# heat1q/libldpc

Measured on AMD Instinct MI355X. Metric: decoded frames/s (n=1024 code, 50 BP iters, AWGN), higher is better.
Workload: dtype f64

## Files before the change

include/ldpc_amd.h:

```cpp
#ifndef LDPC_AMD_H
#define LDPC_AMD_H

#include <stdbool.h>
#include <stdint.h>

#ifdef __cplusplus
extern "C" {
#endif

#if defined(__GNUC__)
#pragma GCC visibility push(default)
#endif

typedef struct
{
    bool earlyTerm;
    uint32_t iterations;
    const char *type;
} decoder_param;

typedef struct
{
    uint64_t seed;
    double xRange[3];
// ... 259 lines not shown
int ldpc_hip_mt64(ldpc_hip_ctx *ctx, uint64_t seed, uint64_t first, uint64_t n, uint64_t *out, void *hip_stream);

int ldpc_hip_selftest_division(ldpc_hip_ctx *ctx, uint64_t n, uint64_t seed, uint64_t *mismatches);

int ldpc_hip_selftest_math(ldpc_hip_ctx *ctx, int fn, uint64_t n, const double *a, const double *b, double *out);

uint64_t ldpc_hip_selftest_chunk_table(uint64_t first_chunk, uint64_t chunks_per_request, uint64_t n_requests, uint64_t gap);
uint64_t ldpc_hip_selftest_shard_table(int world, int rank, uint32_t piece_chunks, uint64_t steps, uint64_t *launches);
uint64_t ldpc_hip_jump_tasks(const ldpc_hip_ctx *ctx);

int ldpc_hip_simulate(ldpc_hip_ctx *ctx, decoder_param dec, channel_param ch, simulation_param sim,
                      sim_results_t *results, uint64_t *totals, bool *stopFlag, int cli_output);

typedef struct ldpc_hip_comm ldpc_hip_comm;

int ldpc_hip_comm_unique_id(uint8_t id[128]);
ldpc_hip_comm *ldpc_hip_comm_create(int rank, int world, int device, const uint8_t id[128]);
ldpc_hip_comm *ldpc_hip_comm_create_shm(int rank, int world, const char *name);
ldpc_hip_comm *ldpc_hip_comm_create_echo(int rank, int world);
void ldpc_hip_comm_destroy(ldpc_hip_comm *comm);
int ldpc_hip_comm_allgather(ldpc_hip_comm *comm, const void *send, void *recv, uint64_t bytes);
void ldpc_hip_fused_plan_info(const ldpc_hip_ctx *ctx, int64_t info[8]);
int ldpc_hip_fused_program(const ldpc_hip_ctx *ctx);
int ldpc_hip_decode_stages(const ldpc_hip_ctx *ctx, decoder_param dec, int32_t stages[3]);
int ldpc_hip_decoder_choice(const ldpc_hip_ctx *ctx, decoder_param dec);
int ldpc_hip_selftest_sim_fold(const uint32_t *iters, const uint32_t *bit_errors, uint64_t n, const uint64_t *ends,
                               uint64_t n_ranges, int world, uint64_t min_fec, uint64_t max_frames, uint64_t out[8]);
int ldpc_hip_selftest_layer_plan(ldpc_hip_ctx *ctx, int32_t *step_of_row);
int ldpc_hip_selftest_place(ldpc_hip_comm *comm, uint64_t nct, uint64_t pairs_before, uint64_t frame_pos, uint64_t cap,
                            uint64_t piece_pairs, uint64_t pairs_with_margin, uint64_t status, uint64_t out[5]);
void ldpc_hip_comm_stats(ldpc_hip_comm *comm, double out[4], int reset);
const char *ldpc_hip_comm_describe(ldpc_hip_comm *comm);

uint64_t ldpc_hip_shard_capacity(const ldpc_hip_ctx *ctx, uint64_t target_frames, int world);
int ldpc_hip_stream_decode_sharded(ldpc_hip_ctx *ctx, ldpc_hip_comm *comm, decoder_param dec, uint64_t target_frames,
                                   const ldpc_hip_out *out, uint64_t step[4], void *hip_stream);
int ldpc_hip_simulate_sharded(ldpc_hip_ctx *ctx, ldpc_hip_comm *comm, decoder_param dec, channel_param ch,
                              simulation_param sim, sim_results_t *results, uint64_t *totals, bool *stopFlag,
                              int cli_output);

#if defined(__GNUC__)
#pragma GCC visibility pop
#endif

#ifdef __cplusplus
}
// ... 3 lines not shown
```

libldpc_amd/binding.py:

```python
import ctypes as ct
import os

import numpy as np

PKG = os.path.dirname(os.path.abspath(__file__))
LIB_PATH = os.environ.get("LDPC_AMD_LIB") or os.path.join(PKG, "libldpc.so")

AWGN, BSC, BEC = 1, 2, 3
CHANNELS = {"AWGN": AWGN, "BSC": BSC, "BEC": BEC}


class decoder_param(ct.Structure):
    _fields_ = [("earlyTerm", ct.c_bool), ("iterations", ct.c_uint32), ("type", ct.c_char_p)]


class channel_param(ct.Structure):
    _fields_ = [("seed", ct.c_uint64), ("xRange", ct.c_double * 3), ("type", ct.c_char_p)]


class simulation_param(ct.Structure):
    _fields_ = [("threads", ct.c_uint32), ("maxFrames", ct.c_uint64), ("fec", ct.c_uint64),
                ("resultFile", ct.c_char_p)]


# ... 148 lines not shown
    L.ldpc_hip_synchronize.argtypes = [vp, vp]
    L.ldpc_hip_batch_counters.restype = i32
    L.ldpc_hip_batch_counters.argtypes = [vp, vp, vp, u64, ct.c_uint32, i32, vp, vp]
    L.ldpc_hip_selftest_division.restype = i32
    L.ldpc_hip_selftest_division.argtypes = [vp, u64, u64, vp]
    L.ldpc_hip_mt64.restype = i32
    L.ldpc_hip_mt64.argtypes = [vp, u64, u64, u64, vp, vp]
    L.ldpc_hip_set_profiling.argtypes = [vp, i32]
    L.ldpc_hip_last_ms.restype = ct.c_float
    L.ldpc_hip_last_ms.argtypes = [vp, i32]
    L.ldpc_hip_comm_unique_id.restype = i32
    L.ldpc_hip_comm_unique_id.argtypes = [vp]
    L.ldpc_hip_comm_create.restype = vp
    L.ldpc_hip_comm_create.argtypes = [i32, i32, i32, vp]
    L.ldpc_hip_comm_create_shm.restype = vp
    L.ldpc_hip_comm_create_shm.argtypes = [i32, i32, ct.c_char_p]
    L.ldpc_hip_comm_create_echo.restype = vp
    L.ldpc_hip_comm_create_echo.argtypes = [i32, i32]
    L.ldpc_hip_comm_destroy.argtypes = [vp]
    L.ldpc_hip_comm_allgather.restype = i32
    L.ldpc_hip_comm_allgather.argtypes = [vp, vp, vp, u64]
    L.ldpc_hip_fused_plan_info.restype = None
    L.ldpc_hip_fused_plan_info.argtypes = [vp, vp]
    L.ldpc_hip_fused_program.restype = i32
    L.ldpc_hip_fused_program.argtypes = [vp]
    L.ldpc_hip_decode_stages.restype = i32
    L.ldpc_hip_decode_stages.argtypes = [vp, decoder_param, vp]
    L.ldpc_hip_decoder_choice.restype = i32
    L.ldpc_hip_decoder_choice.argtypes = [vp, decoder_param]
    L.ldpc_hip_selftest_sim_fold.restype = i32
    L.ldpc_hip_selftest_sim_fold.argtypes = [vp, vp, u64, vp, u64, i32, u64, u64, vp]
    L.ldpc_hip_selftest_layer_plan.restype = i32
    L.ldpc_hip_selftest_layer_plan.argtypes = [vp, vp]
    L.ldpc_hip_selftest_place.restype = i32
    L.ldpc_hip_selftest_place.argtypes = [vp, u64, u64, u64, u64, u64, u64, u64, vp]
    L.ldpc_hip_comm_stats.restype = None
    L.ldpc_hip_comm_stats.argtypes = [vp, vp, i32]
    L.ldpc_hip_comm_describe.restype = ct.c_char_p
    L.ldpc_hip_comm_describe.argtypes = [vp]
    L.ldpc_hip_shard_capacity.restype = u64
    L.ldpc_hip_shard_capacity.argtypes = [vp, u64, i32]
    L.ldpc_hip_stream_decode_sharded.restype = i32
    L.ldpc_hip_stream_decode_sharded.argtypes = [vp, vp, decoder_param, u64, ct.POINTER(ldpc_hip_out), vp, vp]
    L.ldpc_hip_simulate_sharded.restype = i32
    L.ldpc_hip_simulate_sharded.argtypes = [vp, vp, decoder_param, channel_param, simulation_param, ct.POINTER(sim_results_t),
                                            vp, ct.POINTER(ct.c_bool), i32]
# ... 114 lines not shown
            self.ctx = None

    __del__ = close

    def _check(self, rc, what):
        if rc != 0:
            raise RuntimeError(f"{what}: " + self.lib.ldpc_hip_last_error().decode())

    def _outs(self, n, want, out):
        bufs = dict(out or {})
        for name in want:
            if name not in bufs:
                dt, per_bit = self.OUT_SPEC[name]
                bufs[name] = np.zeros((n, self.nc) if per_bit else (n,), dt)
        s = ldpc_hip_out(*[_ptr(bufs.get(k)) for k in ("iters", "bit_errors", "hard", "llr_out", "llr_in", "codeword")])
        return s, bufs

    def set_bec_compat(self, on):
        self.lib.ldpc_hip_set_bec_compat(self.ctx, int(on))

    def fused_plan(self):
        info = (ct.c_int64 * 8)()
        self.lib.ldpc_hip_fused_plan_info(self.ctx, info)
        return dict(zip(("ok", "n_slots", "vnb", "cnl", "small", "calls_stride", "has_shortened", "table_entries"), [int(v) for v in info]))

    def fused_program(self):
        return int(self.lib.ldpc_hip_fused_program(self.ctx))

    STAGES = ("whole", "ratio-first", "ratio-separate", "list-chain", "llr-redo", "handover-first", "handover-resume")

    def decode_stages(self, early_term=True, iterations=50, decoding="BP"):
        stages = (ct.c_int32 * 3)()
        n = self.lib.ldpc_hip_decode_stages(self.ctx, _dec(early_term, iterations, decoding), stages)
        return [self.STAGES[stages[i]] for i in range(n)]

    DECODERS = ("resident", "fast32", "layered32", "layered16", "layered-min-sum", "quantized-min-sum", "ternary",
                "layered-fixed-min-sum")

    def decoder_choice(self, early_term=True, iterations=50, decoding="BP"):
        return self.DECODERS[self.lib.ldpc_hip_decoder_choice(self.ctx, _dec(early_term, iterations, decoding))]

    def set_fast_mode(self, on):
        self.lib.ldpc_hip_set_fast_mode(self.ctx, int(on))

    NOISE_MODES = {"reference": 0, "counter": 1}

    def set_noise(self, mode):
# ... 524 lines not shown
```

libldpc_amd/csrc/api.cpp:

```cpp
#include "../../include/ldpc_amd.h"

#include <hip/hip_runtime.h>

#include <algorithm>
#include <cstdio>
#include <cstdlib>
#include <cstring>
#include <iostream>
#include <memory>
#include <string>
#include <vector>

#include "engine.hpp"
#include "shard_place.hpp"
#include "sim.hpp"
#include "sim_fold.hpp"

using namespace ldpc_amd;

struct ldpc_hip_comm
{
    std::unique_ptr<Comm> comm;
    std::string description;
};
// ... 872 lines not shown
    return c;
}

void ldpc_hip_comm_destroy(ldpc_hip_comm *comm) { delete comm; }

int ldpc_hip_comm_allgather(ldpc_hip_comm *comm, const void *send, void *recv, uint64_t bytes)
{
    return guarded([&] { comm->comm->all_gather(send, recv, bytes); });
}

void ldpc_hip_fused_plan_info(const ldpc_hip_ctx *ctx, int64_t info[8])
{
    const FusedPlan &f = ctx->eng->fused_plan();
    info[0] = f.ok ? 1 : 0, info[1] = f.n_slots, info[2] = f.vnb, info[3] = f.cnl, info[4] = f.wide_exclusive ? 1 : 0;
    info[5] = f.calls_stride, info[6] = f.has_shortened ? 1 : 0, info[7] = static_cast<int64_t>(f.vn_slot.size());
}

int ldpc_hip_fused_program(const ldpc_hip_ctx *ctx)
{
    const FusedPlan &f = ctx->eng->fused_plan();
    return f.ok ? f.program : -1;
}

int ldpc_hip_decode_stages(const ldpc_hip_ctx *ctx, decoder_param dec, int32_t stages[3])
{
    const StageSeq seq = ctx->eng->stages(to_params(dec));
    for (int i = 0; i < seq.n; ++i)
        stages[i] = static_cast<int32_t>(seq.s[i]);
    return seq.n;
}

int ldpc_hip_decoder_choice(const ldpc_hip_ctx *ctx, decoder_param dec) { return static_cast<int>(ctx->eng->decoder(to_params(dec))); }

int ldpc_hip_selftest_layer_plan(ldpc_hip_ctx *ctx, int32_t *step_of_row)
{
    if (!step_of_row)
        return ctx->eng->layer_plan_builds();
    int n = -1;
    if (guarded([&] {
            const LayerPlan &L = ctx->eng->layer_plan();
            if (!L.ok)
                throw std::runtime_error("the layered schedule does not take this code");
            for (size_t i = 0; i < L.step_of_row.size(); ++i)
                step_of_row[i] = L.step_of_row[i];
            n = static_cast<int>(L.steps.size());
        }) != 0)
// ... 101 lines not shown
```

libldpc_amd/csrc/fused_program.hpp:

```cpp
#pragma once

#include <cstdint>

#include "plan.hpp"

namespace ldpc_amd
{

constexpr int kFusedProgCalls = 2;

struct FusedProgCall
{
    int degree, leaf, nm;
    uint32_t cnt0, cnt1;
    uint32_t off0, off1;
    constexpr bool two() const { return cnt1 != 0; }
    constexpr uint32_t flip() const { return ((1u << nm) - 1u) << (degree - leaf - nm); }
    constexpr uint32_t cls() const { return static_cast<uint32_t>(degree) | (static_cast<uint32_t>(leaf) << 3) | (flip() << 4); }
    constexpr FusedCall call() const { return cnt0 ? FusedCall{off0 | (off1 << 16), cnt0 | (cnt1 << 16), cls(), 0} : FusedCall{0, 0, 0, 0}; }
    constexpr bool valid() const { return cnt0 == 0 || (cnt0 <= kWaveSize && (cnt1 == 0 || (cnt0 == kWaveSize && cnt1 == kWaveSize))); }
};

struct FusedProgWave
{
    FusedProgCall leaf;
    FusedProgCall calls[kFusedProgCalls];
    uint32_t vn_kind[4], vn_cnt[4], vn_deg[4];
    constexpr uint32_t vn_prog() const { return vn_kind[0] | (vn_kind[1] << 4) | (vn_kind[2] << 8) | (vn_kind[3] << 12); }
    constexpr uint32_t vn_desc(int s) const { return vn_kind[s] == kFusedVnNone ? 0u : (vn_cnt[s] | (vn_deg[s] << 16)); }
};

struct FusedProgram
{
    int n_slots, vnb, cnl;
    FusedProgWave wave[kDecodeWaves];
};

namespace fused_program_detail
{
constexpr uint32_t kB = kWaveSize * 8u;
constexpr FusedProgCall pair(int d, int leaf, int nm, uint32_t first_slot_byte)
{
    return FusedProgCall{d, leaf, nm, kWaveSize, kWaveSize, first_slot_byte, first_slot_byte + static_cast<uint32_t>(d - leaf) * kB};
}
constexpr FusedProgCall none() { return FusedProgCall{0, 0, 0, 0, 0, 0, 0}; }
constexpr FusedProgWave wide_wave(FusedProgCall leaf, FusedProgCall rest, uint32_t dv)
{
    return FusedProgWave{leaf, {rest, none()}, {kFusedVnWide, kFusedVnNone, kFusedVnNone, kFusedVnNone}, {kWaveSize, 0, 0, 0}, {dv, 0, 0, 0}};
}
constexpr FusedProgWave pairs_wave(FusedProgCall leaf, FusedProgCall rest)
{
    return FusedProgWave{leaf, {rest, none()}, {kFusedVnPair, kFusedVnPair, kFusedVnPair, kFusedVnPair}, {kWaveSize, kWaveSize, kWaveSize, kWaveSize}, {2, 2, 2, 2}};
}
}

constexpr FusedProgram kFusedPrograms[] = {
    {2944, 4, 1,
     {fused_program_detail::wide_wave(fused_program_detail::pair(4, 1, 0, 2048), fused_program_detail::pair(3, 0, 2, 14336), 15),
      fused_program_detail::wide_wave(fused_program_detail::pair(4, 1, 0, 5120), fused_program_detail::pair(3, 0, 2, 17408), 15),
      fused_program_detail::pairs_wave(fused_program_detail::pair(4, 1, 0, 8192), fused_program_detail::pair(3, 0, 2, 20480)),
      fused_program_detail::pairs_wave(fused_program_detail::pair(3, 1, 0, 0), fused_program_detail::pair(3, 0, 2, 11264))}},
};
constexpr int kNumFusedPrograms = static_cast<int>(sizeof(kFusedPrograms) / sizeof(kFusedPrograms[0]));

constexpr bool fused_program_valid(const FusedProgram &p)
{
    if (p.vnb > 4 || p.cnl > 1 || static_cast<uint32_t>(p.n_slots) * 8u > 0x10000u)
        return false;
    for (const FusedProgWave &w : p.wave)
    {
        if (!w.leaf.valid() || (w.leaf.cnt0 != 0 && (w.leaf.leaf != 1 || w.leaf.degree < 3 || w.leaf.degree > 4)))
            return false;
        for (const FusedProgCall &c : w.calls)
            if (!c.valid() || (c.cnt0 != 0 && (c.leaf != 0 || c.degree < 2 || c.degree > 4)))
                return false;
        const bool wide = w.vn_kind[0] == kFusedVnWide;
        for (int s = 0; s < 4; ++s)
        {
            const uint32_t k = w.vn_kind[s];
            if (k == kFusedVnWide ? (s != 0 || w.vn_deg[s] < 3 || w.vn_deg[s] > 15 || w.vn_cnt[s] == 0 || w.vn_cnt[s] > kWaveSize)
                                  : (k == kFusedVnPair ? (w.vn_deg[s] != 2 || w.vn_cnt[s] != kWaveSize || w.vn_kind[s ^ 1] != kFusedVnPair)
                                                       : (k == kFusedVn2 ? (w.vn_deg[s] != 2 || w.vn_cnt[s] == 0 || w.vn_cnt[s] >= kWaveSize) : k != kFusedVnNone)))
                return false;
            if (wide && s > 0 && k != kFusedVnNone)
// ... 18 lines not shown
```

libldpc_amd/csrc/kernels_fused.hip:

```cpp
#include <hip/hip_runtime.h>

#include <algorithm>
#include <utility>

#include "device_cn.hpp"
#include "device_math.hpp"
#include "device_philox.hpp"
#include "fused_program.hpp"
#include "fused_rule.h"
#include "kernels.hpp"
#include "launch_lds.hpp"

#ifndef LDPC_AMD_DECODE_PRIO
#define LDPC_AMD_DECODE_PRIO 3
#endif
#ifndef LDPC_AMD_FUSED_WAVES
#define LDPC_AMD_FUSED_WAVES 6
#endif

namespace ldpc_amd
{

namespace
{

constexpr int kThreads = kDecodeWaves * kWaveSize;

__device__ __forceinline__ double *at(char *msg, uint32_t byte_off) { return reinterpret_cast<double *>(msg + byte_off); }

struct Track
{
    uint32_t hmax, hmin, pmax;
};
__device__ __forceinline__ void track(Track &t, double a)
{
    t.hmax = max(t.hmax, hi_word(a));
    t.hmin = min(t.hmin, hi_word(a));
}
__device__ __forceinline__ void track2(Track &t, double a, double b)
{
    t.hmax = max(max(t.hmax, hi_word(a)), hi_word(b));
    t.hmin = min(min(t.hmin, hi_word(a)), hi_word(b));
}

template <int D, bool LEAF, unsigned FLIP, bool TWO, bool WANT_TOT, bool SHARED = true>
__device__ __forceinline__ uint32_t cnf_call(char *msg, uint32_t off0, uint32_t off1, uint32_t cnt0, int lane, double rho0, double rho1,
                                             uint32_t prev0, uint32_t prev1, uint32_t &lb0, uint32_t &lb1, Track &t, double &tot0,
                                             double &tot1)
{
    constexpr int M = D - (LEAF ? 1 : 0);
    const uint32_t stride = TWO ? kWaveSize * 8u : cnt0 * 8u;
// ... 622 lines not shown
            else
            {
                if (k01 & 0xFu)
                    one(w, k01 & 0xFu);
                if (k01 >> 4)
                    one(w + 1, k01 >> 4);
            }
        }
        vn_bits = bits;
    };
    [[maybe_unused]] auto prog_cn = [&]<int W, int C>() {
        if constexpr (PROG >= 0)
        {
            constexpr FusedProgCall k = C < 0 ? kFusedPrograms[PROG].wave[W].leaf : kFusedPrograms[PROG].wave[W].calls[C];
            if constexpr (k.cnt0 != 0)
            {
                constexpr bool LEAF = C < 0;
                uint32_t lb0 = 0, lb1 = 0, par = 0;
                double tot0 = 1.0, tot1 = 1.0;
                const uint32_t prev0 = LEAF ? leaf_bits << 31 : 0u, prev1 = LEAF ? leaf_bits << 30 : 0u;
                const double rho0 = LEAF ? leaf_rho[0] : 0.0, rho1 = LEAF ? leaf_rho[1] : 0.0;
                if constexpr (k.two())
                    par = cnf_call<k.degree, LEAF, k.flip(), true, false>(msg, k.off0, k.off1, k.cnt0, lane, rho0, rho1, prev0, prev1, lb0, lb1, t, tot0, tot1);
                else if (lane < static_cast<int>(k.cnt0))
                    par = cnf_call<k.degree, LEAF, k.flip(), false, false>(msg, k.off0, 0, k.cnt0, lane, rho0, rho1, prev0, prev1, lb0, lb1, t, tot0, tot1);
                bad |= par;
                if constexpr (LEAF)
                    new_leaf_bits |= lb0 | (lb1 << 1);
            }
        }
    };
    [[maybe_unused]] auto prog_cn_wave = [&]<int W>() { prog_cn.template operator()<W, -1>(), prog_cn.template operator()<W, 0>(), prog_cn.template operator()<W, 1>(); };
    [[maybe_unused]] auto prog_vn2 = [&]<int W, int S>() {
        if constexpr (PROG >= 0)
        {
            constexpr FusedProgWave pw = kFusedPrograms[PROG].wave[W];
            if constexpr (pw.vn_kind[S] == kFusedVnPair && pw.vn_kind[S + 1] == kFusedVnPair)
            {
                uint32_t sga, sgb;
                double ta, tb;
                vn2_pair(msg, idx_at(S), idx_at(S + 1), val_at(S), val_at(S + 1), t, sga, sgb, ta, tb);
                bits |= ((sga >> 31) << S) | ((sgb >> 31) << (S + 1));
            }
            else
            {
#pragma unroll
                for (int s = S; s < S + 2; ++s)
// ... 131 lines not shown
                    }
                };
                for (int c = 0; c < CNL; ++c)
                    if ((leaf_calls_now[4 * c + 1] & 0xFFFFu) != 0)
                        ho_call(leaf_calls_now[4 * c], leaf_calls_now[4 * c + 1], leaf_calls_now[4 * c + 2], c);
                for (int c = 0; c < F.calls_stride; ++c)
                {
                    if ((my_calls[4 * c + 1] & 0xFFFFu) == 0)
                        break;
                    ho_call(my_calls[4 * c], my_calls[4 * c + 1], my_calls[4 * c + 2], 0);
                }
                return;
            }
            cn_pass();
            commit_leaves();
            __syncthreads();
            vn_pass();
            post_vote(I + 1);
            __syncthreads();
            ++I;
        }
    }
    else
    for (;;)
    {
        loop_cn_pass();
        const int ph = I & 1;
        const bool esc = dm_box_escaped(t.hmax, t.hmin) || t.pmax >= DM_FUSED_P_HI;
        const int wave_vote = (__ballot((bad & 0x80000000u) != 0) != 0) | ((__ballot(esc) != 0) << 1);
        if (lane == 0)
            votes[ph][wave] = wave_vote;
        __syncthreads();
        int any = 0;
#pragma unroll
        for (int w = 0; w < kDecodeWaves; ++w)
            any |= votes[ph][w];
        if (any & 2)
        {
            if (tid == 0)
            {
                const uint32_t pos = atomicAdd(a.redo_count, 1u);
                a.redo_list[pos] = static_cast<uint32_t>(frame);
            }
            return;
        }
        if (I > 0 && a.early_term && !(any & 1))
        {
            --I;
            break;
        }
        if (I == a.iterations)
            break;
        commit_leaves();

        loop_vn_pass();
        __syncthreads();
        ++I;
    }

    if (tid == 0 && a.iters)
        a.iters[frame] = I;
    uint8_t *hard = a.hard ? a.hard + frame * nc : nullptr;
    int err = 0;
    if (hard || a.bit_errors)
    {
        int lane_now = lane;
        asm volatile("" : "+v"(lane_now));
        const uint32_t *tab = F.lane_tab + (static_cast<uint32_t>(wave) * kFusedLaneRows) * kWaveSize + lane_now;
        auto account = [&](uint32_t cwd, uint32_t bit) {
            if (cwd == kFusedNone)
                return;
            const uint32_t col = cwd & 0x3FFFFFFFu;
            if (hard)
                hard[col] = static_cast<uint8_t>(bit);
            if (cwd & kFusedCounted)
                err += static_cast<int>(bit) != (cw ? static_cast<int>(cw[col]) : 0);
        };
#pragma unroll
        for (int w = 0; w < VNB; ++w)
            account(tab[(24 + w) * kWaveSize], (vn_bits >> w) & 1u);
// ... 501 lines not shown
```

libldpc_amd/csrc/plan.cpp:

```cpp
#include "plan.hpp"

#include "fused_program.hpp"
#include "fused_rule.h"

#include <algorithm>
#include <cstdio>
#include <cstdlib>
#include <map>
#include <numeric>
#include <stdexcept>

#ifndef LDPC_AMD_FUSED_PROGRAM
#define LDPC_AMD_FUSED_PROGRAM 1
#endif

namespace ldpc_amd
{

namespace
{
void deal(const std::vector<int> &cost, std::vector<uint32_t> &work, int &stride)
{
    std::vector<int> order(cost.size());
    std::iota(order.begin(), order.end(), 0);
// ... 403 lines not shown
        }
    }
    r.uniform_cn = std::all_of(r.cn_deg.begin(), r.cn_deg.end(), [&](uint8_t d) { return d == maxd; });
    r.uniform_vn = nv0 >= 2 && nv1 >= 2;
    for (int rd = 0; rd < 2 && r.uniform_vn; ++rd)
    {
        const int nvr = rd ? nv1 : nv0;
        auto blk = [&](int q) -> const Reg2VnBlock & { return r.vn_blocks[static_cast<size_t>(q / W + (rd ? nv0 : 0)) * W + q % W]; };
        const Reg2VnBlock &b0 = blk(0), &b1 = blk(1);
        uint32_t *af = r.vn_affine[rd];
        af[0] = b0.p0_off, af[1] = b1.p0_off - b0.p0_off, af[2] = b0.prest_off, af[3] = b1.prest_off - b0.prest_off;
        af[4] = b0.tot_off, af[5] = b1.tot_off - b0.tot_off;
        for (int q = 0; q < nvr * W && r.uniform_vn; ++q)
        {
            const Reg2VnBlock &b = blk(q);
            r.uniform_vn = b.count == kWaveSize && b.degree == 3 && b.p0_off == af[0] + af[1] * q && b.prest_off == af[2] + af[3] * q &&
                           b.tot_off == af[4] + af[5] * q;
        }
    }
    r.ok = true;
    return r;
}

FusedPlan build_fused_plan(const LdpcCode &code, const Plan &plan)
{
    FusedPlan f;
    const SparseGF2 &H = code.H;
    if (!plan.lds_ok || plan.has_isolated_vn || H.rows <= 0 ||
        !dm_fused_applies(H.rows, H.cols, H.rptr.data(), H.rcol.data(), H.cptr.data()))
        return f;
    const int W = kDecodeWaves;
    static_assert(DM_FUSED_MAX_LEAF_CALLS == kDecodeWaves * kFusedLeafCalls && DM_FUSED_MAX_VN_BLOCKS == kDecodeWaves * kFusedVnSlots,
                  "a code the rule admits has a plan: the oracle decides by the rule alone");
    auto cdeg = [&](int c) { return H.cptr[c + 1] - H.cptr[c]; };

    struct Row
    {
        int row, order[4];
    };
    std::map<unsigned, std::vector<Row>> by_class;
    for (int i = 0; i < H.rows; ++i)
    {
        Row r{i, {0, 0, 0, 0}};
        unsigned flip;
        int leaf;
        const int d = H.rptr[i + 1] - H.rptr[i];
// ... 13 lines not shown
    for (auto &[cls, rows] : by_class)
    {
        const int d = static_cast<int>(cls & 7u), leaf = static_cast<int>((cls >> 3) & 1u), m = d - leaf;
        for (size_t i = 0; i < rows.size(); i += kWaveSize)
        {
            Block b{cls, slot, {}};
            b.rows.assign(rows.begin() + i, rows.begin() + std::min(rows.size(), i + kWaveSize));
            const uint32_t cnt = static_cast<uint32_t>(b.rows.size());
            for (uint32_t l = 0; l < cnt; ++l)
                for (int k = 0; k < m; ++k)
                    f.edge_slot[H.redge[H.rptr[b.rows[l].row] + b.rows[l].order[k]]] = slot + k * cnt + l;
            slot += static_cast<uint32_t>(m) * cnt;
            blocks.push_back(std::move(b));
        }
    }
    f.n_slots = static_cast<int>(slot);
    if (f.n_slots > DM_FUSED_MAX_SLOTS)
        return f;
    f.ho_map.assign(static_cast<size_t>(f.n_slots), 0);
    for (int e = 0; e < plan.nnz; ++e)
        if (f.edge_slot[e] != kNoSlot)
            f.ho_map[f.edge_slot[e]] = plan.edge_slot[e];

    struct Call
    {
        int b0, b1;
        int cost;
        bool leaf;
    };
    auto class_cost = [](unsigned cls) {
        const int d = static_cast<int>(cls & 7u), leaf = static_cast<int>((cls >> 3) & 1u);
        return d == 2 ? 12 : (d == 3 ? (leaf ? 28 : 30) : (leaf ? 45 : 50));
    };
    std::vector<Call> calls;
    for (size_t b = 0; b < blocks.size();)
    {
        const bool pair = b + 1 < blocks.size() && blocks[b + 1].cls == blocks[b].cls && blocks[b].rows.size() == kWaveSize &&
                          blocks[b + 1].rows.size() == kWaveSize;
        const bool leaf = (blocks[b].cls >> 3) & 1u;
        calls.push_back(Call{static_cast<int>(b), pair ? static_cast<int>(b + 1) : -1, class_cost(blocks[b].cls) * (pair ? 2 : 1) + 4, leaf});
        b += pair ? 2 : 1;
    }
    std::vector<std::vector<int>> w_leaf(W), w_rest(W);
    std::vector<long> load(W, 0);
    {
        std::vector<int> order(calls.size());
        std::iota(order.begin(), order.end(), 0);
        std::stable_sort(order.begin(), order.end(), [&](int a, int b) { return calls[a].cost > calls[b].cost; });
        int n_leaf = 0;
        for (const Call &c : calls)
            n_leaf += c.leaf;
        const int leaf_cap = (n_leaf + W - 1) / W;
        if (leaf_cap > kFusedLeafCalls)
            return f;
        for (int ci : order)
            if (calls[ci].leaf)
            {
                int best = -1;
                for (int w = 0; w < W; ++w)
                    if (static_cast<int>(w_leaf[w].size()) < leaf_cap && (best < 0 || load[w] < load[best]))
                        best = w;
                w_leaf[best].push_back(ci);
                load[best] += calls[ci].cost;
            }
        for (int ci : order)
            if (!calls[ci].leaf)
            {
                const int w = static_cast<int>(std::min_element(load.begin(), load.end()) - load.begin());
                w_rest[w].push_back(ci);
                load[w] += calls[ci].cost;
            }
        f.cnl = leaf_cap;
    }
    auto describe = [&](const Call &c) {
        const Block &b0 = blocks[c.b0];
        FusedCall d{b0.off * 8u, static_cast<uint32_t>(b0.rows.size()), b0.cls, 0};
        if (c.b1 >= 0)
        {
            d.offs |= (blocks[c.b1].off * 8u) << 16;
            d.cnts |= static_cast<uint32_t>(blocks[c.b1].rows.size()) << 16;
        }
        return d;
    };
    f.leaf_calls.assign(static_cast<size_t>(W) * kFusedLeafCalls, FusedCall{0, 0, 0, 0});
    f.calls_stride = 1;
    for (int w = 0; w < W; ++w)
        f.calls_stride = std::max(f.calls_stride, static_cast<int>(w_rest[w].size()) + 1);
    f.calls.assign(static_cast<size_t>(W) * f.calls_stride, FusedCall{0, 0, 0, 0});
    for (int w = 0; w < W; ++w)
    {
        for (size_t i = 0; i < w_leaf[w].size(); ++i)
            f.leaf_calls[static_cast<size_t>(w) * kFusedLeafCalls + i] = describe(calls[w_leaf[w][i]]);
        for (size_t i = 0; i < w_rest[w].size(); ++i)
            f.calls[static_cast<size_t>(w) * f.calls_stride + i] = describe(calls[w_rest[w][i]]);
    }

    std::vector<int> cols;
    for (int c = 0; c < H.cols; ++c)
        if (cdeg(c) >= 2)
            cols.push_back(c);
    std::stable_sort(cols.begin(), cols.end(), [&](int a, int b) { return cdeg(a) > cdeg(b); });
    struct VBlock
    {
        int degree;
        std::vector<int> cols;
    };
    std::vector<VBlock> vblocks;
    for (size_t i = 0; i < cols.size();)
    {
        size_t j = i;
        while (j < cols.size() && j - i < kWaveSize && cdeg(cols[j]) == cdeg(cols[i]))
            ++j;
        vblocks.push_back(VBlock{cdeg(cols[i]), std::vector<int>(cols.begin() + i, cols.begin() + j)});
        i = j;
    }
    std::vector<std::vector<int>> w_vn(W);
    {
        std::vector<int> order(vblocks.size());
        std::iota(order.begin(), order.end(), 0);
        auto cost = [&](int b) { return vblocks[b].degree == 2 ? 13 : 5 * vblocks[b].degree + 8; };
        std::stable_sort(order.begin(), order.end(), [&](int a, int b) { return cost(a) > cost(b); });
        std::vector<long> vload(W, 0);
        for (int b : order)
        {
            int best = -1;
            for (int w = 0; w < W; ++w)
                if (static_cast<int>(w_vn[w].size()) < kFusedVnSlots - 1 && (best < 0 || vload[w] < vload[best]))
                    best = w;
            if (best < 0)
                for (int w = 0; w < W; ++w)
                    if (static_cast<int>(w_vn[w].size()) < kFusedVnSlots && (best < 0 || vload[w] < vload[best]))
                        best = w;
            if (best < 0)
                return f;
            w_vn[best].push_back(b);
            vload[best] += cost(b);
        }
    }
    std::vector<uint32_t> col_entry(H.cols, static_cast<uint32_t>(plan.nct) + 1u), col_word(H.cols);
    for (int c = 0; c < H.cols; ++c)
        col_word[c] = static_cast<uint32_t>(c);
    for (int i = 0; i < static_cast<int>(code.bit_pos.size()); ++i)
    {
        if (i < plan.nct)
            col_entry[code.bit_pos[i]] = static_cast<uint32_t>(i);
        col_word[code.bit_pos[i]] |= kFusedCounted;
    }
    for (int c : code.shorten)
        if (c >= 0 && c < H.cols && plan.rank_kind[plan.col_rank[c]] == 2)
            col_entry[c] = static_cast<uint32_t>(plan.nct);
    f.has_shortened = !code.shorten.empty();
    for (int c = 0; c < H.cols; ++c)
        if (cdeg(c) >= 3 && col_entry[c] <= static_cast<uint32_t>(plan.nct))
            f.need_lambda = true;

    f.vn_desc.assign(static_cast<size_t>(W) * kFusedVnSlots * 4, 0);
    f.lane_tab.assign(static_cast<size_t>(W) * kFusedLaneRows * kWaveSize, 0);
    f.vnb = 1;
    for (int w = 0; w < W; ++w)
    {
        uint32_t *tab = &f.lane_tab[static_cast<size_t>(w) * kFusedLaneRows * kWaveSize];
        for (int r = 16; r < 24; ++r)
            std::fill(tab + r * kWaveSize, tab + (r + 1) * kWaveSize, (static_cast<uint32_t>(plan.nct) + 1u) * 16u);
        for (int r = 32; r < 36; ++r)
            std::fill(tab + r * kWaveSize, tab + (r + 1) * kWaveSize, (static_cast<uint32_t>(plan.nct) + 1u) * 16u);
        for (int r = 24; r < 32; ++r)
            std::fill(tab + r * kWaveSize, tab + (r + 1) * kWaveSize, kFusedNone);
        for (int r = 36; r < 40; ++r)
            std::fill(tab + r * kWaveSize, tab + (r + 1) * kWaveSize, kFusedNone);
        for (int r = 40; r < 44; ++r)
            std::fill(tab + r * kWaveSize, tab + (r + 1) * kWaveSize, 0u);
        std::vector<int> &mine = w_vn[w];
        std::stable_sort(mine.begin(), mine.end(), [&](int a, int b) { return vblocks[a].degree > vblocks[b].degree; });
        std::vector<int> slots;
        for (int b : mine)
        {
            if (vblocks[b].degree == 2 && slots.size() % 2 == 1 && !slots.empty() && slots.back() >= 0 && vblocks[slots.back()].degree != 2 &&
                mine.size() + 1 <= static_cast<size_t>(kFusedVnSlots))
                slots.push_back(-1);
            slots.push_back(b);
        }
        if (static_cast<int>(slots.size()) > kFusedVnSlots)
            return f;
        f.vnb = std::max(f.vnb, static_cast<int>(slots.size()));
        for (size_t sw = 0; sw < slots.size(); ++sw)
        {
            if (slots[sw] < 0)
                continue;
            const VBlock &vb = vblocks[slots[sw]];
            const uint32_t cnt = static_cast<uint32_t>(vb.cols.size());
            uint32_t *d = &f.vn_desc[(static_cast<size_t>(w) * kFusedVnSlots + sw) * 4];
            d[0] = cnt | (static_cast<uint32_t>(vb.degree) << 16);
            d[1] = static_cast<uint32_t>(f.vn_slot.size());
            auto eslot = [&](int l, int p) { return f.edge_slot[H.cedge[H.cptr[vb.cols[l]] + p]] * 8u; };
            const bool in_regs = vb.degree == 2 || (sw == 0 && vb.degree <= 15);
            f.vn_prog[w] |= (vb.degree == 2 ? (cnt == kWaveSize ? kFusedVnPair : kFusedVn2) : (in_regs ? kFusedVnWide : kFusedVnTable)) << (4 * sw);
            if (!in_regs)
                for (int p = 0; p < vb.degree; ++p)
                    for (uint32_t l = 0; l < cnt; ++l)
                        f.vn_slot.push_back(eslot(static_cast<int>(l), p));
            for (uint32_t l = 0; l < cnt; ++l)
            {
                if (vb.degree == 2)
                    tab[sw * kWaveSize + l] = eslot(l, 0) | (eslot(l, 1) << 16);
                else if (in_regs)
                    for (int q = 0; q < vb.degree; ++q)
                        tab[(8 + q / 2) * kWaveSize + l] |= eslot(l, q) << (16 * (q & 1));
                tab[(16 + sw) * kWaveSize + l] = col_entry[vb.cols[l]] * 16u;
                tab[(24 + sw) * kWaveSize + l] = col_word[vb.cols[l]];
            }
        }
        for (size_t c = 0; c < w_leaf[w].size(); ++c)
            for (int h = 0; h < 2; ++h)
            {
                const int bi = h == 0 ? calls[w_leaf[w][c]].b0 : calls[w_leaf[w][c]].b1;
                if (bi < 0)
                    continue;
                const Block &b = blocks[bi];
                const int d = static_cast<int>(b.cls & 7u);
// ... 161 lines not shown
```

libldpc_amd/csrc/plan.hpp:

```cpp
#pragma once

#include <algorithm>
#include <cstdint>
#include <vector>

#include "code.hpp"

namespace ldpc_amd
{

constexpr int kWaveSize = 64;
constexpr int kMaxLdsCnDegree = 8;
constexpr int kMaxCnDegree = 16;
constexpr uint32_t kNoSlot = 0xFFFFFFFFu;
constexpr int kDecodeWaves = 4;

struct CnBlock
{
    uint32_t off;
    uint16_t count;
    uint16_t degree;
};

constexpr int kVnPackedRows = 32;
// ... 163 lines not shown
    uint32_t offs;
    uint32_t cnts;
    uint32_t cls;
    uint32_t pad;
};
struct FusedPlan
{
    bool ok = false;
    int n_slots = 0;
    int vnb = 0, cnl = 0;
    bool has_shortened = false;
    bool need_lambda = false;
    bool wide_exclusive = false;
    int program = -1;
    std::vector<FusedCall> leaf_calls;
    std::vector<FusedCall> calls;
    int calls_stride = 0;
    std::vector<uint32_t> vn_desc;
    uint32_t vn_prog[kDecodeWaves] = {0, 0, 0, 0};
    std::vector<uint32_t> vn_slot;
    std::vector<uint32_t> lane_tab;
    std::vector<uint32_t> edge_slot;
    std::vector<uint32_t> ho_map;
};
constexpr uint32_t kFusedCounted = 0x80000000u, kFusedNone = 0xFFFFFFFFu;
enum : uint32_t { kFusedVnNone = 0, kFusedVnPair = 1 , kFusedVn2 = 2 , kFusedVnWide = 3 , kFusedVnTable = 4 };
FusedPlan build_fused_plan(const LdpcCode &code, const Plan &plan);

Plan build_plan(const LdpcCode &code);
Reg2Plan build_reg2_plan(const LdpcCode &code, const Plan &plan, int nt, int kc, int maxd, int nv0, int nv1);
RegPlan build_reg_plan(const LdpcCode &code, const Plan &plan, int nt, int kc, int maxd, uint32_t lds_budget);

}
```

Before: 24.92 million.

## Balance fused decoder waves jointly over CN and VN costs with pair splitting

Reworks how check-node calls and variable-node blocks are dealt across the four waves of the fused decoder. VN blocks are now assigned first using measured per-kind cost tables, and their load seeds the CN assignment. A new pass splits paired CN calls into singles when that lowers the busiest wave's load. The hard-coded fused program for the n=1024 code is updated to the new layout with single calls. Also adds a plan-inspection API and an optional phase-timer trace that is compiled out by default. The risk is that the cost tables don't match real timing, and single calls may run less efficiently than paired ones.

```diff
diff --git a/include/ldpc_amd.h b/include/ldpc_amd.h
--- a/include/ldpc_amd.h
+++ b/include/ldpc_amd.h
@@ -305,6 +305,7 @@
 int ldpc_hip_comm_allgather(ldpc_hip_comm *comm, const void *send, void *recv, uint64_t bytes);
 void ldpc_hip_fused_plan_info(const ldpc_hip_ctx *ctx, int64_t info[8]);
 int ldpc_hip_fused_program(const ldpc_hip_ctx *ctx);
+int64_t ldpc_hip_fused_plan_deal(const ldpc_hip_ctx *ctx, int64_t *out, int64_t cap);
 int ldpc_hip_decode_stages(const ldpc_hip_ctx *ctx, decoder_param dec, int32_t stages[3]);
 int ldpc_hip_decoder_choice(const ldpc_hip_ctx *ctx, decoder_param dec);
 int ldpc_hip_selftest_sim_fold(const uint32_t *iters, const uint32_t *bit_errors, uint64_t n, const uint64_t *ends,
diff --git a/libldpc_amd/binding.py b/libldpc_amd/binding.py
--- a/libldpc_amd/binding.py
+++ b/libldpc_amd/binding.py
@@ -194,6 +194,9 @@
     L.ldpc_hip_comm_allgather.argtypes = [vp, vp, vp, u64]
     L.ldpc_hip_fused_plan_info.restype = None
     L.ldpc_hip_fused_plan_info.argtypes = [vp, vp]
+    if hasattr(L, "ldpc_hip_fused_plan_deal"):
+        L.ldpc_hip_fused_plan_deal.restype = ct.c_int64
+        L.ldpc_hip_fused_plan_deal.argtypes = [vp, vp, ct.c_int64]
     L.ldpc_hip_fused_program.restype = i32
     L.ldpc_hip_fused_program.argtypes = [vp]
     L.ldpc_hip_decode_stages.restype = i32
@@ -354,7 +357,32 @@
     def fused_plan(self):
         info = (ct.c_int64 * 8)()
         self.lib.ldpc_hip_fused_plan_info(self.ctx, info)
-        return dict(zip(("ok", "n_slots", "vnb", "cnl", "small", "calls_stride", "has_shortened", "table_entries"), [int(v) for v in info]))
+        plan = dict(zip(("ok", "n_slots", "vnb", "cnl", "small", "calls_stride", "has_shortened", "table_entries"), [int(v) for v in info]))
+        plan.update(self._fused_deal())
+        return plan
+
+    VN_KINDS = {1: "pair", 2: "two", 3: "wide", 4: "table"}
+
+    def _fused_deal(self):
+        need = int(self.lib.ldpc_hip_fused_plan_deal(self.ctx, None, 0)) if hasattr(self.lib, "ldpc_hip_fused_plan_deal") else 0
+        if need == 0:
+            return {"cn_blocks": 0, "vn_blocks": 0, "waves": []}
+        buf = (ct.c_int64 * need)()
+        assert int(self.lib.ldpc_hip_fused_plan_deal(self.ctx, buf, need)) == need
+        v = [int(x) for x in buf]
+        n_calls, n_vn = v[2], v[3]
+        waves = [{"cn_load": v[4 + 2 * w], "vn_load": v[5 + 2 * w], "calls": [], "vn": []} for w in range(4)]
+        at = 12
+        for _ in range(n_calls):
+            w, cls, b0, b1, leaf, split, cost, _pad = v[at:at + 8]
+            waves[w]["calls"].append({"cls": cls, "degree": cls & 7, "leaf": leaf, "blocks": [b0] if b1 < 0 else [b0, b1],
+                                      "pair": b1 >= 0, "split": split, "cost": cost})
+            at += 8
+        for _ in range(n_vn):
+            w, slot, block, kind, degree, nodes = v[at:at + 6]
+            waves[w]["vn"].append({"slot": slot, "block": block, "kind": self.VN_KINDS[kind], "degree": degree, "nodes": nodes})
+            at += 6
+        return {"cn_blocks": v[0], "vn_blocks": v[1], "waves": waves}
 
     def fused_program(self):
         return int(self.lib.ldpc_hip_fused_program(self.ctx))
diff --git a/libldpc_amd/csrc/api.cpp b/libldpc_amd/csrc/api.cpp
--- a/libldpc_amd/csrc/api.cpp
+++ b/libldpc_amd/csrc/api.cpp
@@ -918,6 +918,25 @@
     return f.ok ? f.program : -1;
 }
 
+int64_t ldpc_hip_fused_plan_deal(const ldpc_hip_ctx *ctx, int64_t *out, int64_t cap)
+{
+    const FusedPlan &f = ctx->eng->fused_plan();
+    if (!f.ok)
+        return 0;
+    const int64_t need = 4 + 2 * kDecodeWaves + 8 * static_cast<int64_t>(f.deal_calls.size()) + 6 * static_cast<int64_t>(f.deal_vn.size());
+    if (!out || cap < need)
+        return need;
+    int64_t *o = out;
+    *o++ = f.cn_blocks, *o++ = f.vn_blocks, *o++ = static_cast<int64_t>(f.deal_calls.size()), *o++ = static_cast<int64_t>(f.deal_vn.size());
+    for (int w = 0; w < kDecodeWaves; ++w)
+        *o++ = f.cn_load[w], *o++ = f.vn_load[w];
+    for (const FusedPlan::DealCall &c : f.deal_calls)
+        *o++ = c.wave, *o++ = c.cls, *o++ = c.b0, *o++ = c.b1, *o++ = c.leaf ? 1 : 0, *o++ = c.split ? 1 : 0, *o++ = c.cost, *o++ = 0;
+    for (const FusedPlan::DealVn &v : f.deal_vn)
+        *o++ = v.wave, *o++ = v.slot, *o++ = v.block, *o++ = v.kind, *o++ = v.degree, *o++ = v.nodes;
+    return need;
+}
+
 int ldpc_hip_decode_stages(const ldpc_hip_ctx *ctx, decoder_param dec, int32_t stages[3])
 {
     const StageSeq seq = ctx->eng->stages(to_params(dec));
diff --git a/libldpc_amd/csrc/fused_program.hpp b/libldpc_amd/csrc/fused_program.hpp
--- a/libldpc_amd/csrc/fused_program.hpp
+++ b/libldpc_amd/csrc/fused_program.hpp
@@ -43,23 +43,27 @@
 {
     return FusedProgCall{d, leaf, nm, kWaveSize, kWaveSize, first_slot_byte, first_slot_byte + static_cast<uint32_t>(d - leaf) * kB};
 }
+constexpr FusedProgCall single(int d, int leaf, int nm, uint32_t first_slot_byte)
+{
+    return FusedProgCall{d, leaf, nm, kWaveSize, 0, first_slot_byte, 0};
+}
 constexpr FusedProgCall none() { return FusedProgCall{0, 0, 0, 0, 0, 0, 0}; }
-constexpr FusedProgWave wide_wave(FusedProgCall leaf, FusedProgCall rest, uint32_t dv)
+constexpr FusedProgWave wide_wave(FusedProgCall leaf, FusedProgCall c0, FusedProgCall c1, uint32_t dv)
 {
-    return FusedProgWave{leaf, {rest, none()}, {kFusedVnWide, kFusedVnNone, kFusedVnNone, kFusedVnNone}, {kWaveSize, 0, 0, 0}, {dv, 0, 0, 0}};
+    return FusedProgWave{leaf, {c0, c1}, {kFusedVnWide, kFusedVnNone, kFusedVnNone, kFusedVnNone}, {kWaveSize, 0, 0, 0}, {dv, 0, 0, 0}};
 }
-constexpr FusedProgWave pairs_wave(FusedProgCall leaf, FusedProgCall rest)
+constexpr FusedProgWave pairs_wave(FusedProgCall leaf, FusedProgCall c0, FusedProgCall c1)
 {
-    return FusedProgWave{leaf, {rest, none()}, {kFusedVnPair, kFusedVnPair, kFusedVnPair, kFusedVnPair}, {kWaveSize, kWaveSize, kWaveSize, kWaveSize}, {2, 2, 2, 2}};
+    return FusedProgWave{leaf, {c0, c1}, {kFusedVnPair, kFusedVnPair, kFusedVnPair, kFusedVnPair}, {kWaveSize, kWaveSize, kWaveSize, kWaveSize}, {2, 2, 2, 2}};
 }
 }
 
 constexpr FusedProgram kFusedPrograms[] = {
     {2944, 4, 1,
-     {fused_program_detail::wide_wave(fused_program_detail::pair(4, 1, 0, 2048), fused_program_detail::pair(3, 0, 2, 14336), 15),
-      fused_program_detail::wide_wave(fused_program_detail::pair(4, 1, 0, 5120), fused_program_detail::pair(3, 0, 2, 17408), 15),
-      fused_program_detail::pairs_wave(fused_program_detail::pair(4, 1, 0, 8192), fused_program_detail::pair(3, 0, 2, 20480)),
-      fused_program_detail::pairs_wave(fused_program_detail::pair(3, 1, 0, 0), fused_program_detail::pair(3, 0, 2, 11264))}},
+     {fused_program_detail::wide_wave(fused_program_detail::pair(4, 1, 0, 8192), fused_program_detail::single(3, 0, 2, 20480), fused_program_detail::none(), 15),
+      fused_program_detail::wide_wave(fused_program_detail::pair(3, 1, 0, 0), fused_program_detail::pair(3, 0, 2, 17408), fused_program_detail::none(), 15),
+      fused_program_detail::pairs_wave(fused_program_detail::pair(4, 1, 0, 2048), fused_program_detail::pair(3, 0, 2, 11264), fused_program_detail::single(3, 0, 2, 22016)),
+      fused_program_detail::pairs_wave(fused_program_detail::pair(4, 1, 0, 5120), fused_program_detail::pair(3, 0, 2, 14336), fused_program_detail::none())}},
 };
 constexpr int kNumFusedPrograms = static_cast<int>(sizeof(kFusedPrograms) / sizeof(kFusedPrograms[0]));
 
diff --git a/libldpc_amd/csrc/kernels_fused.hip b/libldpc_amd/csrc/kernels_fused.hip
--- a/libldpc_amd/csrc/kernels_fused.hip
+++ b/libldpc_amd/csrc/kernels_fused.hip
@@ -27,6 +27,19 @@
 constexpr int kThreads = kDecodeWaves * kWaveSize;
 
 __device__ __forceinline__ double *at(char *msg, uint32_t byte_off) { return reinterpret_cast<double *>(msg + byte_off); }
+
+#ifdef LDPC_AMD_PHASE_TRACE
+#define FUSED_PHASE_TIMERS uint64_t tr_cn = 0, tr_w1 = 0, tr_vn = 0, tr_w2 = 0, tr_t = __builtin_amdgcn_s_memtime();
+#define FUSED_PHASE_TICK(acc)                             \
+    {                                                     \
+        const uint64_t n_ = __builtin_amdgcn_s_memtime(); \
+        acc += n_ - tr_t;                                 \
+        tr_t = n_;                                        \
+    }
+#else
+#define FUSED_PHASE_TIMERS
+#define FUSED_PHASE_TICK(acc)
+#endif
 
 struct Track
 {
@@ -695,7 +708,7 @@
                 const double rho0 = LEAF ? leaf_rho[0] : 0.0, rho1 = LEAF ? leaf_rho[1] : 0.0;
                 if constexpr (k.two())
                     par = cnf_call<k.degree, LEAF, k.flip(), true, false>(msg, k.off0, k.off1, k.cnt0, lane, rho0, rho1, prev0, prev1, lb0, lb1, t, tot0, tot1);
-                else if (lane < static_cast<int>(k.cnt0))
+                else if (k.cnt0 == kWaveSize || lane < static_cast<int>(k.cnt0))
                     par = cnf_call<k.degree, LEAF, k.flip(), false, false>(msg, k.off0, 0, k.cnt0, lane, rho0, rho1, prev0, prev1, lb0, lb1, t, tot0, tot1);
                 bad |= par;
                 if constexpr (LEAF)
@@ -873,15 +886,19 @@
         }
     }
     else
+    {
+    FUSED_PHASE_TIMERS
     for (;;)
     {
         loop_cn_pass();
+        FUSED_PHASE_TICK(tr_cn)
         const int ph = I & 1;
         const bool esc = dm_box_escaped(t.hmax, t.hmin) || t.pmax >= DM_FUSED_P_HI;
         const int wave_vote = (__ballot((bad & 0x80000000u) != 0) != 0) | ((__ballot(esc) != 0) << 1);
         if (lane == 0)
             votes[ph][wave] = wave_vote;
         __syncthreads();
+        FUSED_PHASE_TICK(tr_w1)
         int any = 0;
 #pragma unroll
         for (int w = 0; w < kDecodeWaves; ++w)
@@ -905,8 +922,18 @@
         commit_leaves();
 
         loop_vn_pass();
+        FUSED_PHASE_TICK(tr_vn)
         __syncthreads();
+        FUSED_PHASE_TICK(tr_w2)
         ++I;
+    }
+#ifdef LDPC_AMD_PHASE_TRACE
+    if (a.phase_trace && frame >= 30000 && frame < 32048 && lane == 0)
+    {
+        uint64_t *o = a.phase_trace + ((frame - 30000) * 4 + wave) * 8;
+        o[0] = tr_cn, o[1] = tr_w1, o[2] = tr_vn, o[3] = tr_w2;
+    }
+#endif
     }
 
     if (tid == 0 && a.iters)
diff --git a/libldpc_amd/csrc/plan.cpp b/libldpc_amd/csrc/plan.cpp
--- a/libldpc_amd/csrc/plan.cpp
+++ b/libldpc_amd/csrc/plan.cpp
@@ -449,6 +449,44 @@
     return r;
 }
 
+namespace
+{
+struct FusedCosts
+{
+    int cn_pair[5][2], cn_single[5][2];
+    int cn2_flip_pair, cn2_flip_single;
+    int vn2_pair, vn2_single;
+    int wide[16];
+    int table_base, table_per_edge;
+};
+constexpr FusedCosts kFusedCosts = {
+    {{0, 0}, {0, 0}, {14, 14}, {52, 47}, {86, 79}},
+    {{0, 0}, {0, 0}, {9, 9}, {31, 28}, {47, 44}},
+    14, 7,
+    27, 15,
+    {0, 0, 0, 33, 36, 41, 49, 54, 60, 65, 71, 76, 84, 89, 95, 101},
+    25, 10,
+};
+int fused_cn_cost(unsigned cls, bool pair)
+{
+    const int d = static_cast<int>(cls & 7u), leaf = static_cast<int>((cls >> 3) & 1u);
+    int c = (pair ? kFusedCosts.cn_pair : kFusedCosts.cn_single)[d][leaf];
+    if (d == 2)
+        c += __builtin_popcount(cls >> 4) * (pair ? kFusedCosts.cn2_flip_pair : kFusedCosts.cn2_flip_single);
+    return c;
+}
+int fused_vn_cost(uint32_t kind, int degree)
+{
+    switch (kind)
+    {
+    case kFusedVnPair: return (kFusedCosts.vn2_pair + 1) / 2;
+    case kFusedVn2: return kFusedCosts.vn2_single;
+    case kFusedVnWide: return kFusedCosts.wide[degree];
+    default: return kFusedCosts.table_base + kFusedCosts.table_per_edge * degree;
+    }
+}
+}
+
 FusedPlan build_fused_plan(const LdpcCode &code, const Plan &plan)
 {
     FusedPlan f;
@@ -508,15 +546,91 @@
         if (f.edge_slot[e] != kNoSlot)
             f.ho_map[f.edge_slot[e]] = plan.edge_slot[e];
 
+    std::vector<int> cols;
+    for (int c = 0; c < H.cols; ++c)
+        if (cdeg(c) >= 2)
+            cols.push_back(c);
+    std::stable_sort(cols.begin(), cols.end(), [&](int a, int b) { return cdeg(a) > cdeg(b); });
+    struct VBlock
+    {
+        int degree;
+        std::vector<int> cols;
+    };
+    std::vector<VBlock> vblocks;
+    for (size_t i = 0; i < cols.size();)
+    {
+        size_t j = i;
+        while (j < cols.size() && j - i < kWaveSize && cdeg(cols[j]) == cdeg(cols[i]))
+            ++j;
+        vblocks.push_back(VBlock{cdeg(cols[i]), std::vector<int>(cols.begin() + i, cols.begin() + j)});
+        i = j;
+    }
+    auto vn_kind = [&](const VBlock &vb, size_t slot) -> uint32_t {
+        if (vb.degree == 2)
+            return vb.cols.size() == kWaveSize ? kFusedVnPair : kFusedVn2;
+        return slot == 0 && vb.degree <= 15 ? kFusedVnWide : kFusedVnTable;
+    };
+    std::vector<std::vector<int>> w_vn(W);
+    {
+        std::vector<long> vload(W, 0);
+        for (int b = 0; b < static_cast<int>(vblocks.size()); ++b)
+        {
+            int best = -1;
+            for (int w = 0; w < W; ++w)
+                if (static_cast<int>(w_vn[w].size()) < kFusedVnSlots - 1 && (best < 0 || vload[w] < vload[best]))
+                    best = w;
+            if (best < 0)
+                for (int w = 0; w < W; ++w)
+                    if (static_cast<int>(w_vn[w].size()) < kFusedVnSlots && (best < 0 || vload[w] < vload[best]))
+                        best = w;
+            if (best < 0)
+                return f;
+            vload[best] += fused_vn_cost(vn_kind(vblocks[b], w_vn[best].size()), vblocks[b].degree);
+            w_vn[best].push_back(b);
+        }
+    }
+    std::vector<std::vector<int>> w_slots(W);
+    f.vnb = 1;
+    f.vn_blocks = static_cast<int>(vblocks.size());
+    for (int w = 0; w < W; ++w)
+    {
+        const std::vector<int> &mine = w_vn[w];
+        std::vector<int> &slots = w_slots[w];
+        for (int b : mine)
+        {
+            if (vblocks[b].degree == 2 && slots.size() % 2 == 1 && !slots.empty() && slots.back() >= 0 && vblocks[slots.back()].degree != 2 &&
+                mine.size() + 1 <= static_cast<size_t>(kFusedVnSlots))
+                slots.push_back(-1);
+            slots.push_back(b);
+        }
+        if (static_cast<int>(slots.size()) > kFusedVnSlots)
+            return f;
+        f.vnb = std::max(f.vnb, static_cast<int>(slots.size()));
+        for (size_t sw = 0; sw < slots.size(); ++sw)
+            if (slots[sw] >= 0)
+            {
+                const VBlock &vb = vblocks[slots[sw]];
+                const uint32_t kind = vn_kind(vb, sw);
+                f.vn_prog[w] |= kind << (4 * sw);
+                f.deal_vn.push_back(FusedPlan::DealVn{w, static_cast<int>(sw), slots[sw], vb.degree, static_cast<int>(vb.cols.size()), kind});
+            }
+        for (size_t sw = 0; sw < slots.size(); ++sw)
+            if (slots[sw] >= 0)
+            {
+                const uint32_t kind = (f.vn_prog[w] >> (4 * sw)) & 0xFu;
+                const bool lock_step = kind == kFusedVnPair && ((f.vn_prog[w] >> (4 * (sw ^ 1))) & 0xFu) == kFusedVnPair;
+                if (lock_step)
+                    f.vn_load[w] += (sw & 1) ? 0 : kFusedCosts.vn2_pair;
+                else
+                    f.vn_load[w] += fused_vn_cost(kind == kFusedVnPair ? static_cast<uint32_t>(kFusedVn2) : kind, vblocks[slots[sw]].degree);
+            }
+    }
+
     struct Call
     {
         int b0, b1;
         int cost;
-        bool leaf;
-    };
-    auto class_cost = [](unsigned cls) {
-        const int d = static_cast<int>(cls & 7u), leaf = static_cast<int>((cls >> 3) & 1u);
-        return d == 2 ? 12 : (d == 3 ? (leaf ? 28 : 30) : (leaf ? 45 : 50));
+        bool leaf, split;
     };
     std::vector<Call> calls;
     for (size_t b = 0; b < blocks.size();)
@@ -524,11 +638,12 @@
         const bool pair = b + 1 < blocks.size() && blocks[b + 1].cls == blocks[b].cls && blocks[b].rows.size() == kWaveSize &&
                           blocks[b + 1].rows.size() == kWaveSize;
         const bool leaf = (blocks[b].cls >> 3) & 1u;
-        calls.push_back(Call{static_cast<int>(b), pair ? static_cast<int>(b + 1) : -1, class_cost(blocks[b].cls) * (pair ? 2 : 1) + 4, leaf});
+        calls.push_back(Call{static_cast<int>(b), pair ? static_cast<int>(b + 1) : -1, fused_cn_cost(blocks[b].cls, pair), leaf, false});
         b += pair ? 2 : 1;
     }
+    f.cn_blocks = static_cast<int>(blocks.size());
     std::vector<std::vector<int>> w_leaf(W), w_rest(W);
-    std::vector<long> load(W, 0);
+    std::vector<long> load(f.vn_load, f.vn_load + W);
     {
         std::vector<int> order(calls.size());
         std::iota(order.begin(), order.end(), 0);
@@ -557,6 +672,46 @@
                 load[w] += calls[ci].cost;
             }
         f.cnl = leaf_cap;
+        for (size_t round = calls.size(); round > 0; --round)
+        {
+            const int w = static_cast<int>(std::max_element(load.begin(), load.end()) - load.begin());
+            bool split = false;
+            for (size_t i = 0; i < w_rest[w].size() && !split; ++i)
+            {
+                const int ci = w_rest[w][i];
+                const Call c = calls[ci];
+                if (c.b1 < 0)
+                    continue;
+                const int single = fused_cn_cost(blocks[c.b0].cls, false);
+                std::vector<long> trial = load;
+                trial[w] -= c.cost;
+                const int t0 = static_cast<int>(std::min_element(trial.begin(), trial.end()) - trial.begin());
+                trial[t0] += single;
+                const int t1 = static_cast<int>(std::min_element(trial.begin(), trial.end()) - trial.begin());
+                trial[t1] += single;
+                if (*std::max_element(trial.begin(), trial.end()) >= load[w])
+                    continue;
+                w_rest[w].erase(w_rest[w].begin() + static_cast<std::ptrdiff_t>(i));
+                calls[ci] = Call{c.b0, -1, single, false, true};
+                w_rest[t0].push_back(ci);
+                calls.push_back(Call{c.b1, -1, single, false, true});
+                w_rest[t1].push_back(static_cast<int>(calls.size()) - 1);
+                load = trial;
+                split = true;
+            }
+            if (!split)
+                break;
+        }
+    }
+    for (int w = 0; w < W; ++w)
+    {
+        auto note = [&](int ci) {
+            const Call &c = calls[ci];
+            f.deal_calls.push_back(FusedPlan::DealCall{w, c.b0, c.b1, blocks[c.b0].cls, c.cost, c.leaf, c.split});
+            f.cn_load[w] += c.cost;
+        };
+        std::for_each(w_leaf[w].begin(), w_leaf[w].end(), note);
+        std::for_each(w_rest[w].begin(), w_rest[w].end(), note);
     }
     auto describe = [&](const Call &c) {
         const Block &b0 = blocks[c.b0];
@@ -581,48 +736,6 @@
             f.calls[static_cast<size_t>(w) * f.calls_stride + i] = describe(calls[w_rest[w][i]]);
     }
 
-    std::vector<int> cols;
-    for (int c = 0; c < H.cols; ++c)
-        if (cdeg(c) >= 2)
-            cols.push_back(c);
-    std::stable_sort(cols.begin(), cols.end(), [&](int a, int b) { return cdeg(a) > cdeg(b); });
-    struct VBlock
-    {
-        int degree;
-        std::vector<int> cols;
-    };
-    std::vector<VBlock> vblocks;
-    for (size_t i = 0; i < cols.size();)
-    {
-        size_t j = i;
-        while (j < cols.size() && j - i < kWaveSize && cdeg(cols[j]) == cdeg(cols[i]))
-            ++j;
-        vblocks.push_back(VBlock{cdeg(cols[i]), std::vector<int>(cols.begin() + i, cols.begin() + j)});
-        i = j;
-    }
-    std::vector<std::vector<int>> w_vn(W);
-    {
-        std::vector<int> order(vblocks.size());
-        std::iota(order.begin(), order.end(), 0);
-        auto cost = [&](int b) { return vblocks[b].degree == 2 ? 13 : 5 * vblocks[b].degree + 8; };
-        std::stable_sort(order.begin(), order.end(), [&](int a, int b) { return cost(a) > cost(b); });
-        std::vector<long> vload(W, 0);
-        for (int b : order)
-        {
-            int best = -1;
-            for (int w = 0; w < W; ++w)
-                if (static_cast<int>(w_vn[w].size()) < kFusedVnSlots - 1 && (best < 0 || vload[w] < vload[best]))
-                    best = w;
-            if (best < 0)
-                for (int w = 0; w < W; ++w)
-                    if (static_cast<int>(w_vn[w].size()) < kFusedVnSlots && (best < 0 || vload[w] < vload[best]))
-                        best = w;
-            if (best < 0)
-                return f;
-            w_vn[best].push_back(b);
-            vload[best] += cost(b);
-        }
-    }
     std::vector<uint32_t> col_entry(H.cols, static_cast<uint32_t>(plan.nct) + 1u), col_word(H.cols);
     for (int c = 0; c < H.cols; ++c)
         col_word[c] = static_cast<uint32_t>(c);
@@ -642,7 +755,6 @@
 
     f.vn_desc.assign(static_cast<size_t>(W) * kFusedVnSlots * 4, 0);
     f.lane_tab.assign(static_cast<size_t>(W) * kFusedLaneRows * kWaveSize, 0);
-    f.vnb = 1;
     for (int w = 0; w < W; ++w)
     {
         uint32_t *tab = &f.lane_tab[static_cast<size_t>(w) * kFusedLaneRows * kWaveSize];
@@ -656,19 +768,7 @@
             std::fill(tab + r * kWaveSize, tab + (r + 1) * kWaveSize, kFusedNone);
         for (int r = 40; r < 44; ++r)
             std::fill(tab + r * kWaveSize, tab + (r + 1) * kWaveSize, 0u);
-        std::vector<int> &mine = w_vn[w];
-        std::stable_sort(mine.begin(), mine.end(), [&](int a, int b) { return vblocks[a].degree > vblocks[b].degree; });
-        std::vector<int> slots;
-        for (int b : mine)
-        {
-            if (vblocks[b].degree == 2 && slots.size() % 2 == 1 && !slots.empty() && slots.back() >= 0 && vblocks[slots.back()].degree != 2 &&
-                mine.size() + 1 <= static_cast<size_t>(kFusedVnSlots))
-                slots.push_back(-1);
-            slots.push_back(b);
-        }
-        if (static_cast<int>(slots.size()) > kFusedVnSlots)
-            return f;
-        f.vnb = std::max(f.vnb, static_cast<int>(slots.size()));
+        const std::vector<int> &slots = w_slots[w];
         for (size_t sw = 0; sw < slots.size(); ++sw)
         {
             if (slots[sw] < 0)
@@ -680,7 +780,6 @@
             d[1] = static_cast<uint32_t>(f.vn_slot.size());
             auto eslot = [&](int l, int p) { return f.edge_slot[H.cedge[H.cptr[vb.cols[l]] + p]] * 8u; };
             const bool in_regs = vb.degree == 2 || (sw == 0 && vb.degree <= 15);
-            f.vn_prog[w] |= (vb.degree == 2 ? (cnt == kWaveSize ? kFusedVnPair : kFusedVn2) : (in_regs ? kFusedVnWide : kFusedVnTable)) << (4 * sw);
             if (!in_regs)
                 for (int p = 0; p < vb.degree; ++p)
                     for (uint32_t l = 0; l < cnt; ++l)
diff --git a/libldpc_amd/csrc/plan.hpp b/libldpc_amd/csrc/plan.hpp
--- a/libldpc_amd/csrc/plan.hpp
+++ b/libldpc_amd/csrc/plan.hpp
@@ -209,6 +209,22 @@
     std::vector<uint32_t> lane_tab;
     std::vector<uint32_t> edge_slot;
     std::vector<uint32_t> ho_map;
+    struct DealCall
+    {
+        int wave, b0, b1;
+        uint32_t cls;
+        int cost;
+        bool leaf, split;
+    };
+    struct DealVn
+    {
+        int wave, slot, block, degree, nodes;
+        uint32_t kind;
+    };
+    std::vector<DealCall> deal_calls;
+    std::vector<DealVn> deal_vn;
+    int cn_blocks = 0, vn_blocks = 0;
+    long cn_load[kDecodeWaves] = {0, 0, 0, 0}, vn_load[kDecodeWaves] = {0, 0, 0, 0};
 };
 constexpr uint32_t kFusedCounted = 0x80000000u, kFusedNone = 0xFFFFFFFFu;
 enum : uint32_t { kFusedVnNone = 0, kFusedVnPair = 1 , kFusedVn2 = 2 , kFusedVnWide = 3 , kFusedVnTable = 4 };
```

Result: no change. 25.03 million (median of 6 runs) (+0.4%).
